# GabeTsai/YOLO-For-Turbines

Hardware: AMD Instinct MI355X
Metric: images/sec at 416x416 (fwd) (higher is better)
Workload: dtype f32; 1 GPU; BASELINE configs[1]: batch 32/GPU 416x416 fp32 inference, 80-class head, YOLOv3 forward (75 fused conv launches); per_gpu_batch=32, global_batch=32, image_size=416, num_classes=80, parallelism=image-sharded x1 (no collective)

## Files before the change

### yolo_for_turbines_amd/csrc/conv_wino4_f32.hip

```cpp
#include "wino_dma.h"

namespace yolo {

__device__ constexpr float W4_BT[6][6] = {
    {1.f, 1.5f, -2.f, -1.5f, 1.f, 0.f},
    {0.f, -1.f, -2.5f, -0.5f, 1.f, 0.f},
    {0.f, 1.f, 0.5f, -2.5f, 1.f, 0.f},
    {0.f, -0.5f, -1.f, 0.5f, 1.f, 0.f},
    {0.f, 2.f, -1.f, -2.f, 1.f, 0.f},
    {0.f, 1.f, 1.5f, -2.f, -1.5f, 1.f},
};
__device__ constexpr float W4_AT[4][6] = {
    {1.f, 1.f, 1.f, 1.f, 1.f, 0.f},
    {0.f, 1.f, -1.f, 2.f, -0.5f, 0.f},
    {0.f, 1.f, 1.f, 4.f, 0.25f, 0.f},
    {0.f, 1.f, -1.f, 8.f, -0.125f, 1.f},
};
__device__ constexpr double W4_G[6][3] = {
    {1.0, 0.0, 0.0},
    {-1.0 / 3, -1.0 / 3, -1.0 / 3},
    {1.0 / 3, -1.0 / 3, 1.0 / 3},
    {1.0 / 15, 2.0 / 15, 4.0 / 15},
    {-16.0 / 15, 8.0 / 15, -4.0 / 15},
    {0.0, 0.0, 1.0},
};

struct Wino4XArgs {
    const float* x;
    float* V;
    int H, W, C4, C4p;
    int x_ld, x_off;
    int th, tw, T, Tpad;
    int ncg;
    int nxb;
    const float* w;
    float* U;
    int cout, cin, coutp, cinp, kpad;
    long long utotal;
};

__device__ __forceinline__ void wino4_filter_elems(const Wino4XArgs& p, long long first, long long stride) {
    for (long long i = first; i < p.utotal; i += stride) {
        const int e = (int)(i & 3);
        const long long r = i >> 2;
        const int co = (int)(r % p.coutp), c4 = (int)(r / p.coutp);
        const int ci = 4 * c4 + e;
        double g[3][3];
        const bool ok = co < p.cout && ci < p.cin;
#pragma unroll
        for (int k = 0; k < 9; ++k) g[k / 3][k % 3] = ok ? (double)p.w[(size_t)co * p.kpad + k * p.cinp + ci] : 0.0;
        double t[6][3];
#pragma unroll
        for (int j = 0; j < 6; ++j)
#pragma unroll
            for (int q = 0; q < 3; ++q) t[j][q] = W4_G[j][0] * g[0][q] + W4_G[j][1] * g[1][q] + W4_G[j][2] * g[2][q];
        float* dst = p.U + i;
        const size_t xs = (size_t)p.C4p * p.coutp * 4;
#pragma unroll
        for (int j = 0; j < 6; ++j)
#pragma unroll
            for (int l = 0; l < 6; ++l)
                dst[(6 * j + l) * xs] = (float)(t[j][0] * W4_G[l][0] + t[j][1] * W4_G[l][1] + t[j][2] * W4_G[l][2]);
    }
}

__global__ __launch_bounds__(256) void wino4_filters_f32(const Wino4XArgs p) {
    wino4_filter_elems(p, (long long)blockIdx.x * blockDim.x + threadIdx.x, (long long)gridDim.x * blockDim.x);
}

__global__ __launch_bounds__(256) void wino4_xform_f32(const Wino4XArgs p) {
    if ((int)blockIdx.x >= p.nxb) {
        wino4_filter_elems(p, (long long)(blockIdx.x - p.nxb) * blockDim.x + threadIdx.x, (long long)(gridDim.x - p.nxb) * blockDim.x);
        return;
    }
    const int lane = threadIdx.x & 63, wave = threadIdx.x >> 6;
    const int cg = blockIdx.x % p.ncg, tb = blockIdx.x / p.ncg;
    const int c4 = cg * 8 + (lane & 7);
    const int t = tb * 32 + wave * 8 + (lane >> 3);
    if (c4 >= p.C4p) return;
    const bool tv = t < p.T && c4 < p.C4;
    const int tt = t < p.T ? t : 0;
    const int per = p.th * p.tw;
    const int n = tt / per, rem = tt - n * per;
    const int ty = rem / p.tw, tx = rem - ty * p.tw;
    const int r0 = 4 * ty - 1, c0 = 4 * tx - 1;
    const float* base = p.x + p.x_off + 4 * (c4 < p.C4 ? c4 : 0);
    f32x4 v[6][6];
#pragma unroll
    for (int i = 0; i < 6; ++i)
#pragma unroll
        for (int l = 0; l < 6; ++l) v[i][l] = f32x4{0.f, 0.f, 0.f, 0.f};
#pragma unroll
    for (int k = 0; k < 6; ++k) {
        const int r = r0 + k;
        const bool rv = tv && r >= 0 && r < p.H;
        f32x4 d[6];
#pragma unroll
        for (int j = 0; j < 6; ++j) {
            const int c = c0 + j;
            const bool ok = rv && c >= 0 && c < p.W;
            const size_t pix = ok ? ((size_t)n * p.H + r) * p.W + c : 0;
            const f32x4 ld = *reinterpret_cast<const f32x4*>(base + pix * p.x_ld);
            const f32x4 z = {0.f, 0.f, 0.f, 0.f};
            d[j] = ok ? ld : z;
        }
        f32x4 e[6];
#pragma unroll
        for (int l = 0; l < 6; ++l) {
            e[l] = f32x4{0.f, 0.f, 0.f, 0.f};
#pragma unroll
            for (int j = 0; j < 6; ++j)
                if (W4_BT[l][j] != 0.f) e[l] += W4_BT[l][j] * d[j];
        }
#pragma unroll
        for (int i = 0; i < 6; ++i)
            if (W4_BT[i][k] != 0.f)
#pragma unroll
                for (int l = 0; l < 6; ++l) v[i][l] += W4_BT[i][k] * e[l];
    }
    float* dst = p.V + ((size_t)c4 * p.Tpad + t) * 4;
    const size_t xs = (size_t)p.C4p * p.Tpad * 4;
#pragma unroll
    for (int i = 0; i < 6; ++i)
#pragma unroll
        for (int l = 0; l < 6; ++l) *reinterpret_cast<f32x4*>(dst + (6 * i + l) * xs) = v[i][l];
}

struct Wino4Args {
    const float* V;
    const float* U;
    const float* scale;
    const float* shift;
    const float* res;
    float* y;
    int* nan_flag;
    int T, Tpad, C4p, Cout, CoutPad;
    int th, tw, H, W;
    int y_ld, y_off, r_ld, r_off;
    int flags;
    int n_mt, n_nt;
    int n_whole;
};

constexpr int W4_STAGE = 24576;
constexpr int W4_SLOTS = 4;
constexpr int W4_DMA = 3;
constexpr int W4_TAB = 512;

template <int OFF>
__device__ __forceinline__ void w4_read3(float& a, float& b0, float& b1, unsigned ua, unsigned va) {
    asm volatile("ds_read_b32 %0, %1 offset:%2" : "=&v"(a) : "v"(ua), "n"(OFF));
    asm volatile("ds_read_b32 %0, %1 offset:%2" : "=&v"(b0) : "v"(va), "n"(OFF));
    asm volatile("ds_read_b32 %0, %1 offset:%2" : "=&v"(b1) : "v"(va), "n"(OFF + 256));
}

template <int ACT, bool RES>
__global__ __launch_bounds__(512, 1) void conv_wino4_f32(const Wino4Args p) {
    extern __shared__ __attribute__((aligned(16))) char smem[];
    const int tid = threadIdx.x, lane = tid & 63;
    const int wave = __builtin_amdgcn_readfirstlane(tid >> 6);
    const int l16 = lane & 15, kq = lane >> 4;
    const int xcd = blockIdx.x & 7, q = blockIdx.x >> 3;
    const int nt = q % p.n_nt, row = q / p.n_nt;
    const int wrows = (p.n_whole + 7) >> 3;
    const bool cut = row >= wrows;
    const int half = (row - wrows) & 1;
    const int mt = cut ? p.n_whole + ((row - wrows) >> 1) * 8 + xcd : row * 8 + xcd;
    if (mt >= (cut ? p.n_mt : p.n_whole)) return;
    const int wm = cut ? half : wave & 1, wn = cut ? wave & 3 : wave >> 1;
    const bool busy = !cut || wave < 4;

    int* tab = reinterpret_cast<int*>(smem + W4_SLOTS * W4_STAGE);
    if (tid < 64) {
        const int t = mt * 64 + tid;
        const bool tv = t < p.T && (!cut || (tid >> 5) == half);
        const int tt = tv ? t : 0;
        const int per = p.th * p.tw;
        const int n = tt / per, rem = tt - n * per;
        const int ty = rem / p.tw, tx = rem - ty * p.tw;
        const int nr = p.H - 4 * ty < 4 ? p.H - 4 * ty : 4, nc = p.W - 4 * tx < 4 ? p.W - 4 * tx : 4;
        tab[tid] = (n * p.H + 4 * ty) * p.W + 4 * tx;
        tab[64 + tid] = tv ? (nr << 4 | nc) : 0;
    }

    const size_t v_xi = (size_t)p.C4p * p.Tpad * 4, v_c4 = (size_t)p.Tpad * 4;
    const size_t u_xi = (size_t)p.C4p * p.CoutPad * 4, u_c4 = (size_t)p.CoutPad * 4;
    const int grp = wave >> 1, x0 = 3 * (wave & 1);
    const int plane = grp & 1;
    const char* src = grp < 2 ? reinterpret_cast<const char*>(p.V + plane * v_c4 + (size_t)mt * 256)
                              : reinterpret_cast<const char*>(p.U + plane * u_c4 + (size_t)nt * 256);
    const size_t s_xi = (grp < 2 ? v_xi : u_xi) * 4, s_c4 = (grp < 2 ? v_c4 : u_c4) * 4;
    const unsigned lane16 = lane * 16;
    const unsigned lds0 = (unsigned)(size_t)(wn_lptr)smem;
    auto issue_piece = [&](int k, int pass, int st, int slot) {
        const int x = x0 + k;
        wn_glds16_s(src + (size_t)(6 * pass + x) * s_xi + (size_t)(2 * st) * s_c4, lane16, lds0 + slot * W4_STAGE + (6 * grp + x) * 1024);
    };
    auto issue = [&](int pass, int st, int slot) { wn_for<0, W4_DMA>([&](auto K) { issue_piece(decltype(K)::value, pass, st, slot); }); };

    const unsigned vb = lds0 + (32 * wm + l16) * 16 + kq * 4;
    const unsigned ub = lds0 + 12288 + (16 * wn + l16) * 16 + kq * 4;

    const int nst = p.C4p / 2;
    f32x4 py[2][4][4];
#pragma unroll
    for (int bb = 0; bb < 2; ++bb)
#pragma unroll
        for (int i = 0; i < 4; ++i)
#pragma unroll
            for (int j = 0; j < 4; ++j) py[bb][i][j] = f32x4{0.f, 0.f, 0.f, 0.f};

    auto run_pass = [&](auto PASS) {
        constexpr int a = decltype(PASS)::value;
        float fa[12], fb0[12], fb1[12];
        if constexpr (a == 0) {
            issue(0, 0, 0);
            if (nst > 1) issue(0, 1, 1);
            if (nst > 2) issue(0, 2, 2);
        }
        __builtin_amdgcn_sched_barrier(0);
        f32x4 acc[6][2];
#pragma unroll
        for (int x = 0; x < 6; ++x)
#pragma unroll
            for (int bb = 0; bb < 2; ++bb) acc[x][bb] = f32x4{0.f, 0.f, 0.f, 0.f};
#pragma unroll
        for (int x = 0; x < 6; ++x) asm volatile("" : "+v"(acc[x][0]), "+v"(acc[x][1]));
        __builtin_amdgcn_sched_barrier(0);
        if (nst > 2) wn_wait_vmcnt<2 * W4_DMA>();
        else if (nst > 1) wn_wait_vmcnt<W4_DMA>();
        else wn_wait_vmcnt<0>();
        __builtin_amdgcn_s_barrier();
        __builtin_amdgcn_sched_barrier(0);
        w4_read3<0>(fa[0], fb0[0], fb1[0], ub, vb);
        w4_read3<1024>(fa[1], fb0[1], fb1[1], ub, vb);

        int slot = 0;
        for (int st = 0; st < nst; ++st) {
            const unsigned sb = (unsigned)slot * W4_STAGE;
            const int ns = (slot + 1) & (W4_SLOTS - 1);
            const unsigned nb = (unsigned)ns * W4_STAGE;
            wn_for<0, 12>([&](auto S) {
                constexpr int s = decltype(S)::value, x = s % 6;
                if constexpr (s == 10) {
                    __builtin_amdgcn_sched_barrier(0);
                    if (st + 2 < nst) wn_wait_vmcnt<W4_DMA>();
                    else wn_wait_vmcnt<0>();
                    __builtin_amdgcn_s_barrier();
                    __builtin_amdgcn_sched_barrier(0);
                }
                if constexpr (s + 2 < 12) w4_read3<(s + 2) * 1024>(fa[s + 2], fb0[s + 2], fb1[s + 2], ub + sb, vb + sb);
                constexpr int after = s < 10 ? 6 : 3;
                asm volatile("s_waitcnt lgkmcnt(%3)" : "+v"(fa[s]), "+v"(fb0[s]), "+v"(fb1[s]) : "n"(after));
                acc[x][0] = __builtin_amdgcn_mfma_f32_16x16x4f32(fa[s], fb0[s], acc[x][0], 0, 0, 0);
                acc[x][1] = __builtin_amdgcn_mfma_f32_16x16x4f32(fa[s], fb1[s], acc[x][1], 0, 0, 0);
                if constexpr (s < W4_DMA) {
                    __builtin_amdgcn_sched_barrier(0);
                    if (st >= 1 && st + 2 < nst) issue_piece(s, a, st + 2, (slot + 2) & (W4_SLOTS - 1));
                    __builtin_amdgcn_sched_barrier(0);
                }
                if constexpr (s >= 10) {
                    __builtin_amdgcn_sched_barrier(0);
                    w4_read3<(s - 10) * 1024>(fa[s - 10], fb0[s - 10], fb1[s - 10], ub + nb, vb + nb);
                    __builtin_amdgcn_sched_barrier(0);
                }
            });
            slot = ns;
        }
        asm volatile("s_waitcnt lgkmcnt(0)" ::: "memory");
        __syncthreads();
        if constexpr (a < 5) {
            issue(a + 1, 0, 0);
            if (nst > 1) issue(a + 1, 1, 1);
            if (nst > 2) issue(a + 1, 2, 2);
            __builtin_amdgcn_sched_barrier(0);
        }
#pragma unroll
        for (int bb = 0; bb < 2; ++bb) {
            f32x4 mb[6];
#pragma unroll
            for (int b = 0; b < 6; ++b) mb[b] = acc[b][bb];
            f32x4 t[4];
#pragma unroll
            for (int j = 0; j < 4; ++j) {
                t[j] = f32x4{0.f, 0.f, 0.f, 0.f};
#pragma unroll
                for (int b = 0; b < 6; ++b)
                    if (W4_AT[j][b] != 0.f) t[j] += W4_AT[j][b] * mb[b];
            }
#pragma unroll
            for (int i = 0; i < 4; ++i)
                if (W4_AT[i][a] != 0.f)
#pragma unroll
                    for (int j = 0; j < 4; ++j) py[bb][i][j] += W4_AT[i][a] * t[j];
        }
#pragma unroll
        for (int bb = 0; bb < 2; ++bb)
#pragma unroll
            for (int i = 0; i < 4; ++i)
#pragma unroll
                for (int j = 0; j < 4; ++j) asm volatile("" : "+a"(py[bb][i][j]));
    };
    if (busy) {
        run_pass(std::integral_constant<int, 0>{});
        run_pass(std::integral_constant<int, 1>{});
        run_pass(std::integral_constant<int, 2>{});
        run_pass(std::integral_constant<int, 3>{});
        run_pass(std::integral_constant<int, 4>{});
        run_pass(std::integral_constant<int, 5>{});
    } else {
        for (int a = 0; a < 6; ++a) {
            if (a == 0) {
                issue(0, 0, 0);
                if (nst > 1) issue(0, 1, 1);
                if (nst > 2) issue(0, 2, 2);
            }
            if (nst > 2) wn_wait_vmcnt<2 * W4_DMA>();
            else if (nst > 1) wn_wait_vmcnt<W4_DMA>();
            else wn_wait_vmcnt<0>();
            __builtin_amdgcn_s_barrier();
            int slot = 0;
            for (int st = 0; st < nst; ++st) {
                if (st >= 1 && st + 2 < nst) issue(a, st + 2, (slot + 2) & (W4_SLOTS - 1));
                if (st + 2 < nst) wn_wait_vmcnt<W4_DMA>();
                else wn_wait_vmcnt<0>();
                __builtin_amdgcn_s_barrier();
                slot = (slot + 1) & (W4_SLOTS - 1);
            }
            __syncthreads();
            if (a < 5) {
                issue(a + 1, 0, 0);
                if (nst > 1) issue(a + 1, 1, 1);
                if (nst > 2) issue(a + 1, 2, 2);
            }
        }
    }

    constexpr int OLD = 68;
    float* ost = reinterpret_cast<float*>(smem);
    const int c16 = tid & 15;
    const int co_t = nt * 64 + 4 * c16;
    const bool cv = co_t < p.Cout;
    const f32x4 sc_t = *reinterpret_cast<const f32x4*>(p.scale + (cv ? co_t : 0));
    const f32x4 sh_t = *reinterpret_cast<const f32x4*>(p.shift + (cv ? co_t : 0));
    auto row_pixels = [&](int i, int (&pix)[8], bool (&pv)[8]) {
#pragma unroll
        for (int it = 0; it < 8; ++it) {
            const int tl = (tid >> 4) + 32 * (it & 1), j = it >> 1;
            const int fl = tab[64 + tl];
            pv[it] = cv && j < (fl & 15) && i < (fl >> 4);
            pix[it] = pv[it] ? tab[tl] + i * p.W + j : 0;
        }
    };
    auto request_res = [&](const int (&pix)[8], f32x4 (&rr)[8]) {
#pragma unroll
        for (int it = 0; it < 8; ++it)
            rr[it] = *reinterpret_cast<const f32x4*>(p.res + (size_t)pix[it] * p.r_ld + p.r_off + (cv ? co_t : 0));
    };
    f32x4 rr[8];
    if (RES) {
        int pix[8];
        bool pv[8];
        row_pixels(0, pix, pv);
        request_res(pix, rr);
    }
    __builtin_amdgcn_sched_barrier(0);
    bool saw_nan = false;
#pragma unroll
    for (int i = 0; i < 4; ++i) {
        if (i > 0) __syncthreads();
        if (busy) {
            float* dst = ost + (32 * wm + l16) * OLD + 16 * wn + 4 * kq;
#pragma unroll
            for (int bb = 0; bb < 2; ++bb)
#pragma unroll
                for (int j = 0; j < 4; ++j) *reinterpret_cast<f32x4*>(dst + (j * 64 + 16 * bb) * OLD) = py[bb][i][j];
        }
        __syncthreads();
        int pix[8];
        bool pv[8];
        row_pixels(i, pix, pv);
        f32x4 va[8];
#pragma unroll
        for (int it = 0; it < 8; ++it)
            va[it] = *reinterpret_cast<const f32x4*>(ost + ((it >> 1) * 64 + (tid >> 4) + 32 * (it & 1)) * OLD + 4 * c16);
#pragma unroll
        for (int it = 0; it < 8; ++it) {
#pragma unroll
            for (int e = 0; e < 4; ++e) va[it][e] = act_c<ACT>(va[it][e] * sc_t[e] + sh_t[e]);
            if (RES) va[it] += rr[it];
            saw_nan |= pv[it] & ((va[it][0] != va[it][0]) | (va[it][1] != va[it][1]) | (va[it][2] != va[it][2]) | (va[it][3] != va[it][3]));
        }
#pragma unroll
        for (int it = 0; it < 8; ++it) asm volatile("" : "+v"(va[it]));
        if (RES && i < 3) {
            int npix[8];
            bool npv[8];
            row_pixels(i + 1, npix, npv);
            request_res(npix, rr);
            __builtin_amdgcn_sched_barrier(0);
        }
#pragma unroll
        for (int it = 0; it < 8; ++it)
            if (pv[it]) *reinterpret_cast<f32x4*>(p.y + (size_t)pix[it] * p.y_ld + p.y_off + co_t) = va[it];
    }
    if ((p.flags & YOLO_FLAG_NANCHECK) && saw_nan) atomicOr(p.nan_flag, 2);
}

static long long wino4_tiles(const yolo_conv_desc* d) { return (long long)d->n * ((d->h + 3) / 4) * ((d->w + 3) / 4); }

bool wino4_supported(const yolo_conv_desc* d) {
    if (!wino_supported(d)) return false;
    const long long T = wino4_tiles(d);
    if (T + 64 > 0x7fffffffLL / 4) return false;
    const long long C4p = (d->cin / 4 + 1) / 2 * 2, ncg = (C4p + 7) / 8;
    return (T + 63) / 32 * ncg + 1024 <= 0x7fffffffLL;
}

bool wino4_eligible(const yolo_conv_desc* d) {
    if (switches().no_winograd || !wino_eligible(d) || !wino4_supported(d)) return false;
    const long long area = (long long)d->h * d->w, padded = 16LL * ((d->h + 3) / 4) * ((d->w + 3) / 4);
    return area >= 26 * 26 && 5 * padded <= 6 * area;
}

size_t wino4_workspace_bytes(const yolo_conv_desc* d) {
    if (!wino4_supported(d)) return 0;
    const size_t C4p = (size_t)(d->cin / 4 + 1) / 2 * 2;
    const size_t Tpad = (size_t)(wino4_tiles(d) + 63) / 64 * 64;
    const size_t CoutPad = (size_t)round_up(d->cout, 64);
    return 36 * C4p * (Tpad + CoutPad) * 4 * sizeof(float);
}

static int wino4_num_cus() {
    static std::atomic<int> cus[64];
    int dev = 0;
    if (hipGetDevice(&dev) != hipSuccess) { (void)hipGetLastError(); return 0; }
    int n = cus[dev & 63].load(std::memory_order_relaxed);
    if (n > 0) return n;
    if (hipDeviceGetAttribute(&n, hipDeviceAttributeMultiprocessorCount, dev) != hipSuccess || n <= 0) { (void)hipGetLastError(); return 0; }
    cus[dev & 63].store(n, std::memory_order_relaxed);
    return n;
}

static int wino4_whole_blocks(int n_mt, int n_nt, int cus) {
    if (cus <= 0) return n_mt;
    const long long wgs = (long long)n_mt * n_nt;
    const int whole = (int)(wgs / cus * cus / n_nt);
    const long long tail = (long long)(n_mt - whole) * n_nt;
    return tail == 0 || 2 * tail > cus ? n_mt : whole;
}

static void wino4_filter_args(Wino4XArgs& xa, const yolo_conv_desc* d, const float* w_rm, float* U) {
    const int C4p = round_up(d->cin / 4, 2), CoutPad = round_up(d->cout, 64);
    xa.C4p = C4p;
    xa.w = w_rm; xa.U = U; xa.cout = d->cout; xa.cin = d->cin; xa.coutp = CoutPad; xa.cinp = cin_pad_of(d->cin); xa.kpad = kpad_of(d->cin, 3);
    xa.utotal = (long long)C4p * CoutPad * 4;
}
static int wino4_filter_blocks(const Wino4XArgs& xa) {
    const long long ub = (xa.utotal + 255) / 256;
    return (int)(ub < 1024 ? ub : 1024);
}

size_t wino4_filter_bytes(const yolo_conv_desc* d) {
    if (!wino4_supported(d)) return 0;
    return (size_t)36 * round_up(d->cin / 4, 2) * round_up(d->cout, 64) * 4 * sizeof(float);
}

int conv_wino4_launch(const yolo_conv_desc* d, const void* x, const float* w_rm, const float* U4_ready, const float* scale, const float* shift,
                      const void* residual, void* y, void* workspace, size_t workspace_bytes, int32_t* nan_flag, hipStream_t s) {
    if (!wino4_supported(d)) return fail(YOLO_ERR_UNSUPPORTED, "conv winograd F(4x4): needs fp32 3x3 stride 1, NHWC output, channels %% 4 == 0");
    const size_t need = wino4_workspace_bytes(d);
    if (!workspace || workspace_bytes < need) return fail(YOLO_ERR_WORKSPACE, "conv winograd F(4x4): workspace %zu < %zu bytes", workspace_bytes, need);
    if ((size_t)workspace & 15) return fail(YOLO_ERR_ARG, "conv winograd F(4x4): workspace must be 16-byte aligned");
    if ((size_t)U4_ready & 15) return fail(YOLO_ERR_ARG, "conv winograd F(4x4): transformed filters must be 16-byte aligned");
    const int th = (d->h + 3) / 4, tw = (d->w + 3) / 4;
    const int T = d->n * th * tw, Tpad = round_up(T, 64), C4 = d->cin / 4, C4p = round_up(C4, 2);
    const int CoutPad = round_up(d->cout, 64);
    float* V = (float*)workspace;
    float* U = V + (size_t)36 * C4p * Tpad * 4;
    Wino4XArgs xa;
    wino4_filter_args(xa, d, w_rm, U);
    xa.x = (const float*)x; xa.V = V; xa.H = d->h; xa.W = d->w; xa.C4 = C4; xa.x_ld = d->x_ld; xa.x_off = d->x_off;
    xa.th = th; xa.tw = tw; xa.T = T; xa.Tpad = Tpad; xa.ncg = ceil_div(C4p, 8);
    xa.nxb = (Tpad / 32) * xa.ncg;
    const int nub = U4_ready ? 0 : wino4_filter_blocks(xa);
    hipLaunchKernelGGL(wino4_xform_f32, dim3((unsigned)(xa.nxb + nub)), dim3(256), 0, s, xa);
    if (int rc = check_launch("wino4_xform_f32")) return rc;

    Wino4Args a;
    a.V = V; a.U = U4_ready ? U4_ready : U; a.scale = scale; a.shift = shift; a.res = (const float*)residual; a.y = (float*)y;
    a.nan_flag = nan_flag;
    a.T = T; a.Tpad = Tpad; a.C4p = C4p; a.Cout = d->cout; a.CoutPad = CoutPad;
    a.th = th; a.tw = tw; a.H = d->h; a.W = d->w;
    a.y_ld = d->y_ld; a.y_off = d->y_off; a.r_ld = d->r_ld; a.r_off = d->r_off; a.flags = d->flags;
    a.n_mt = Tpad / 64; a.n_nt = CoutPad / 64;
    a.n_whole = wino4_whole_blocks(a.n_mt, a.n_nt, wino4_num_cus());
    const int grid = 8 * a.n_nt * (ceil_div(a.n_whole, 8) + 2 * ceil_div(a.n_mt - a.n_whole, 8));
    const bool res = d->flags & YOLO_FLAG_RESIDUAL;
    const size_t lds = (size_t)W4_SLOTS * W4_STAGE + W4_TAB;
    auto go = [&](auto kern) -> int {
        static LdsOnce once;
        if (int rc = reserve_lds(once, reinterpret_cast<const void*>(kern), lds, "conv_wino4_f32")) return rc;
        hipLaunchKernelGGL(kern, dim3(grid), dim3(512), lds, s, a);
        return check_launch("conv_wino4_f32");
    };
    YOLO_SWITCH_ACT(d->act, return res ? go(&conv_wino4_f32<ACT, true>) : go(&conv_wino4_f32<ACT, false>));
    return fail(YOLO_ERR_ARG, "conv winograd F(4x4): activation");
}

}

extern "C" {

size_t yolo_wino4_filter_bytes(const yolo_conv_desc* d) { return d ? yolo::wino4_filter_bytes(d) : 0; }

int yolo_wino4_filters(const yolo_conv_desc* d, const void* w_packed, void* U4, void* stream) {
    using namespace yolo;
    if (!d || !w_packed || !U4) return fail(YOLO_ERR_ARG, "wino4 filters: null pointer");
    if (!wino4_supported(d)) return fail(YOLO_ERR_UNSUPPORTED, "wino4 filters: needs fp32 3x3 stride 1, NHWC output, channels %% 4 == 0");
    if ((size_t)U4 & 15) return fail(YOLO_ERR_ARG, "wino4 filters: U4 must be 16-byte aligned");
    Wino4XArgs xa{};
    wino4_filter_args(xa, d, (const float*)w_packed, (float*)U4);
    hipLaunchKernelGGL(wino4_filters_f32, dim3((unsigned)wino4_filter_blocks(xa)), dim3(256), 0, (hipStream_t)stream, xa);
    return check_launch("wino4_filters_f32");
}

int yolo_conv_wino4_blocks(const yolo_conv_desc* d, int* whole, int* half) {
    using namespace yolo;
    if (!d || !whole || !half) return fail(YOLO_ERR_ARG, "wino4 blocks: null pointer");
    if (!wino4_supported(d)) return fail(YOLO_ERR_UNSUPPORTED, "wino4 blocks: needs fp32 3x3 stride 1, NHWC output, channels %% 4 == 0");
    const int cus = wino4_num_cus();
    if (cus <= 0) return fail(YOLO_ERR_LAUNCH, "wino4 blocks: no current device");
    const int n_mt = (int)((wino4_tiles(d) + 63) / 64), n_nt = round_up(d->cout, 64) / 64;
    *whole = wino4_whole_blocks(n_mt, n_nt, cus);
    *half = n_mt - *whole;
    return YOLO_OK;
}

}
```

Baseline: 2853 images/s.

## Use all eight waves on cut Winograd F(4,3) tiles with single-column MFMA work

For the partial (cut) M-tiles, the old kernel left four of eight waves idle except for DMA and barrier participation. Now every wave computes a 16-row slice with one MFMA column (NB=1), templating the pass and epilogue on NB. This spreads the 32-tile half across all waves and drops the duplicated idle-wave control path. The cost is extra code instantiation, register pressure from two variants, and lane ids recomputed via mbcnt to limit live ranges.

```diff
diff --git a/yolo_for_turbines_amd/csrc/conv_wino4_f32.hip b/yolo_for_turbines_amd/csrc/conv_wino4_f32.hip
--- a/yolo_for_turbines_amd/csrc/conv_wino4_f32.hip
+++ b/yolo_for_turbines_amd/csrc/conv_wino4_f32.hip
@@ -147,11 +147,11 @@
 constexpr int W4_DMA = 3;
 constexpr int W4_TAB = 512;
 
-template <int OFF>
-__device__ __forceinline__ void w4_read3(float& a, float& b0, float& b1, unsigned ua, unsigned va) {
+template <int OFF, int NB>
+__device__ __forceinline__ void w4_read(float& a, float& b0, float& b1, unsigned ua, unsigned va) {
     asm volatile("ds_read_b32 %0, %1 offset:%2" : "=&v"(a) : "v"(ua), "n"(OFF));
     asm volatile("ds_read_b32 %0, %1 offset:%2" : "=&v"(b0) : "v"(va), "n"(OFF));
-    asm volatile("ds_read_b32 %0, %1 offset:%2" : "=&v"(b1) : "v"(va), "n"(OFF + 256));
+    if constexpr (NB == 2) asm volatile("ds_read_b32 %0, %1 offset:%2" : "=&v"(b1) : "v"(va), "n"(OFF + 256));
 }
 
 template <int ACT, bool RES>
@@ -167,8 +167,7 @@
     const int half = (row - wrows) & 1;
     const int mt = cut ? p.n_whole + ((row - wrows) >> 1) * 8 + xcd : row * 8 + xcd;
     if (mt >= (cut ? p.n_mt : p.n_whole)) return;
-    const int wm = cut ? half : wave & 1, wn = cut ? wave & 3 : wave >> 1;
-    const bool busy = !cut || wave < 4;
+    const int trow = cut ? 32 * half + 16 * (wave >> 2) : 32 * (wave & 1), wn = cut ? wave & 3 : wave >> 1;
 
     int* tab = reinterpret_cast<int*>(smem + W4_SLOTS * W4_STAGE);
     if (tid < 64) {
@@ -190,50 +189,46 @@
     const char* src = grp < 2 ? reinterpret_cast<const char*>(p.V + plane * v_c4 + (size_t)mt * 256)
                               : reinterpret_cast<const char*>(p.U + plane * u_c4 + (size_t)nt * 256);
     const size_t s_xi = (grp < 2 ? v_xi : u_xi) * 4, s_c4 = (grp < 2 ? v_c4 : u_c4) * 4;
-    const unsigned lane16 = lane * 16;
     const unsigned lds0 = (unsigned)(size_t)(wn_lptr)smem;
+    unsigned lane16 = lane * 16;
     auto issue_piece = [&](int k, int pass, int st, int slot) {
         const int x = x0 + k;
         wn_glds16_s(src + (size_t)(6 * pass + x) * s_xi + (size_t)(2 * st) * s_c4, lane16, lds0 + slot * W4_STAGE + (6 * grp + x) * 1024);
     };
     auto issue = [&](int pass, int st, int slot) { wn_for<0, W4_DMA>([&](auto K) { issue_piece(decltype(K)::value, pass, st, slot); }); };
 
-    const unsigned vb = lds0 + (32 * wm + l16) * 16 + kq * 4;
+    const unsigned vb = lds0 + (trow + l16) * 16 + kq * 4;
     const unsigned ub = lds0 + 12288 + (16 * wn + l16) * 16 + kq * 4;
 
     const int nst = p.C4p / 2;
-    f32x4 py[2][4][4];
-#pragma unroll
-    for (int bb = 0; bb < 2; ++bb)
-#pragma unroll
-        for (int i = 0; i < 4; ++i)
-#pragma unroll
-            for (int j = 0; j < 4; ++j) py[bb][i][j] = f32x4{0.f, 0.f, 0.f, 0.f};
-
-    auto run_pass = [&](auto PASS) {
+    auto run_pass = [&](auto PASS, auto& py) {
         constexpr int a = decltype(PASS)::value;
+        constexpr int NB = (int)std::extent<std::remove_reference_t<decltype(py)>>::value;
         float fa[12], fb0[12], fb1[12];
+        lane16 = 16u * __builtin_amdgcn_mbcnt_hi(~0u, __builtin_amdgcn_mbcnt_lo(~0u, 0u));
         if constexpr (a == 0) {
             issue(0, 0, 0);
             if (nst > 1) issue(0, 1, 1);
             if (nst > 2) issue(0, 2, 2);
         }
         __builtin_amdgcn_sched_barrier(0);
-        f32x4 acc[6][2];
+        f32x4 acc[6][NB];
 #pragma unroll
         for (int x = 0; x < 6; ++x)
 #pragma unroll
-            for (int bb = 0; bb < 2; ++bb) acc[x][bb] = f32x4{0.f, 0.f, 0.f, 0.f};
-#pragma unroll
-        for (int x = 0; x < 6; ++x) asm volatile("" : "+v"(acc[x][0]), "+v"(acc[x][1]));
+            for (int bb = 0; bb < NB; ++bb) acc[x][bb] = f32x4{0.f, 0.f, 0.f, 0.f};
+#pragma unroll
+        for (int x = 0; x < 6; ++x)
+#pragma unroll
+            for (int bb = 0; bb < NB; ++bb) asm volatile("" : "+v"(acc[x][bb]));
         __builtin_amdgcn_sched_barrier(0);
         if (nst > 2) wn_wait_vmcnt<2 * W4_DMA>();
         else if (nst > 1) wn_wait_vmcnt<W4_DMA>();
         else wn_wait_vmcnt<0>();
         __builtin_amdgcn_s_barrier();
         __builtin_amdgcn_sched_barrier(0);
-        w4_read3<0>(fa[0], fb0[0], fb1[0], ub, vb);
-        w4_read3<1024>(fa[1], fb0[1], fb1[1], ub, vb);
+        w4_read<0, NB>(fa[0], fb0[0], fb1[0], ub, vb);
+        w4_read<1024, NB>(fa[1], fb0[1], fb1[1], ub, vb);
 
         int slot = 0;
         for (int st = 0; st < nst; ++st) {
@@ -249,11 +244,12 @@
                     __builtin_amdgcn_s_barrier();
                     __builtin_amdgcn_sched_barrier(0);
                 }
-                if constexpr (s + 2 < 12) w4_read3<(s + 2) * 1024>(fa[s + 2], fb0[s + 2], fb1[s + 2], ub + sb, vb + sb);
-                constexpr int after = s < 10 ? 6 : 3;
-                asm volatile("s_waitcnt lgkmcnt(%3)" : "+v"(fa[s]), "+v"(fb0[s]), "+v"(fb1[s]) : "n"(after));
+                if constexpr (s + 2 < 12) w4_read<(s + 2) * 1024, NB>(fa[s + 2], fb0[s + 2], fb1[s + 2], ub + sb, vb + sb);
+                constexpr int after = (s < 10 ? 2 : 1) * (1 + NB);
+                if constexpr (NB == 2) asm volatile("s_waitcnt lgkmcnt(%3)" : "+v"(fa[s]), "+v"(fb0[s]), "+v"(fb1[s]) : "n"(after));
+                else asm volatile("s_waitcnt lgkmcnt(%2)" : "+v"(fa[s]), "+v"(fb0[s]) : "n"(after));
                 acc[x][0] = __builtin_amdgcn_mfma_f32_16x16x4f32(fa[s], fb0[s], acc[x][0], 0, 0, 0);
-                acc[x][1] = __builtin_amdgcn_mfma_f32_16x16x4f32(fa[s], fb1[s], acc[x][1], 0, 0, 0);
+                if constexpr (NB == 2) acc[x][1] = __builtin_amdgcn_mfma_f32_16x16x4f32(fa[s], fb1[s], acc[x][1], 0, 0, 0);
                 if constexpr (s < W4_DMA) {
                     __builtin_amdgcn_sched_barrier(0);
                     if (st >= 1 && st + 2 < nst) issue_piece(s, a, st + 2, (slot + 2) & (W4_SLOTS - 1));
@@ -261,7 +257,7 @@
                 }
                 if constexpr (s >= 10) {
                     __builtin_amdgcn_sched_barrier(0);
-                    w4_read3<(s - 10) * 1024>(fa[s - 10], fb0[s - 10], fb1[s - 10], ub + nb, vb + nb);
+                    w4_read<(s - 10) * 1024, NB>(fa[s - 10], fb0[s - 10], fb1[s - 10], ub + nb, vb + nb);
                     __builtin_amdgcn_sched_barrier(0);
                 }
             });
@@ -276,7 +272,7 @@
             __builtin_amdgcn_sched_barrier(0);
         }
 #pragma unroll
-        for (int bb = 0; bb < 2; ++bb) {
+        for (int bb = 0; bb < NB; ++bb) {
             f32x4 mb[6];
 #pragma unroll
             for (int b = 0; b < 6; ++b) mb[b] = acc[b][bb];
@@ -294,115 +290,107 @@
 #pragma unroll
                     for (int j = 0; j < 4; ++j) py[bb][i][j] += W4_AT[i][a] * t[j];
         }
-#pragma unroll
-        for (int bb = 0; bb < 2; ++bb)
+        if constexpr (a < 5 || NB == 2)
+#pragma unroll
+        for (int bb = 0; bb < NB; ++bb)
 #pragma unroll
             for (int i = 0; i < 4; ++i)
 #pragma unroll
                 for (int j = 0; j < 4; ++j) asm volatile("" : "+a"(py[bb][i][j]));
     };
-    if (busy) {
-        run_pass(std::integral_constant<int, 0>{});
-        run_pass(std::integral_constant<int, 1>{});
-        run_pass(std::integral_constant<int, 2>{});
-        run_pass(std::integral_constant<int, 3>{});
-        run_pass(std::integral_constant<int, 4>{});
-        run_pass(std::integral_constant<int, 5>{});
-    } else {
-        for (int a = 0; a < 6; ++a) {
-            if (a == 0) {
-                issue(0, 0, 0);
-                if (nst > 1) issue(0, 1, 1);
-                if (nst > 2) issue(0, 2, 2);
-            }
-            if (nst > 2) wn_wait_vmcnt<2 * W4_DMA>();
-            else if (nst > 1) wn_wait_vmcnt<W4_DMA>();
-            else wn_wait_vmcnt<0>();
-            __builtin_amdgcn_s_barrier();
-            int slot = 0;
-            for (int st = 0; st < nst; ++st) {
-                if (st >= 1 && st + 2 < nst) issue(a, st + 2, (slot + 2) & (W4_SLOTS - 1));
-                if (st + 2 < nst) wn_wait_vmcnt<W4_DMA>();
-                else wn_wait_vmcnt<0>();
-                __builtin_amdgcn_s_barrier();
-                slot = (slot + 1) & (W4_SLOTS - 1);
-            }
-            __syncthreads();
-            if (a < 5) {
-                issue(a + 1, 0, 0);
-                if (nst > 1) issue(a + 1, 1, 1);
-                if (nst > 2) issue(a + 1, 2, 2);
-            }
-        }
-    }
+    auto run_passes = [&](auto& py) {
+        constexpr int NB = (int)std::extent<std::remove_reference_t<decltype(py)>>::value;
+#pragma unroll
+        for (int bb = 0; bb < NB; ++bb)
+#pragma unroll
+            for (int i = 0; i < 4; ++i)
+#pragma unroll
+                for (int j = 0; j < 4; ++j) py[bb][i][j] = f32x4{0.f, 0.f, 0.f, 0.f};
+        wn_for<0, 6>([&](auto PASS) { run_pass(PASS, py); });
+    };
 
     constexpr int OLD = 68;
     float* ost = reinterpret_cast<float*>(smem);
-    const int c16 = tid & 15;
-    const int co_t = nt * 64 + 4 * c16;
-    const bool cv = co_t < p.Cout;
-    const f32x4 sc_t = *reinterpret_cast<const f32x4*>(p.scale + (cv ? co_t : 0));
-    const f32x4 sh_t = *reinterpret_cast<const f32x4*>(p.shift + (cv ? co_t : 0));
-    auto row_pixels = [&](int i, int (&pix)[8], bool (&pv)[8]) {
-#pragma unroll
-        for (int it = 0; it < 8; ++it) {
-            const int tl = (tid >> 4) + 32 * (it & 1), j = it >> 1;
-            const int fl = tab[64 + tl];
-            pv[it] = cv && j < (fl & 15) && i < (fl >> 4);
-            pix[it] = pv[it] ? tab[tl] + i * p.W + j : 0;
+    bool saw_nan = false;
+    auto epilogue = [&](auto& py) {
+        constexpr int NB = (int)std::extent<std::remove_reference_t<decltype(py)>>::value;
+        constexpr int NIT = 4 * NB;
+        const int lane = __builtin_amdgcn_mbcnt_hi(~0u, __builtin_amdgcn_mbcnt_lo(~0u, 0u));
+        const int tid = wave * 64 + lane, l16 = lane & 15, kq = lane >> 4;
+        const int c16 = tid & 15;
+        const int co_t = nt * 64 + 4 * c16;
+        const bool cv = co_t < p.Cout;
+        const f32x4 sc_t = *reinterpret_cast<const f32x4*>(p.scale + (cv ? co_t : 0));
+        const f32x4 sh_t = *reinterpret_cast<const f32x4*>(p.shift + (cv ? co_t : 0));
+        auto tile_of = [&](int it) { return NB == 2 ? (tid >> 4) + 32 * (it & 1) : (tid >> 4) + 32 * half; };
+        auto pixel_of = [&](int it) { return NB == 2 ? it >> 1 : it; };
+        auto row_pixels = [&](int i, int (&pix)[NIT], bool (&pv)[NIT]) {
+#pragma unroll
+            for (int it = 0; it < NIT; ++it) {
+                const int tl = tile_of(it), j = pixel_of(it);
+                const int fl = tab[64 + tl];
+                pv[it] = cv && j < (fl & 15) && i < (fl >> 4);
+                pix[it] = pv[it] ? tab[tl] + i * p.W + j : 0;
+            }
+        };
+        auto request_res = [&](const int (&pix)[NIT], f32x4 (&rr)[NIT]) {
+#pragma unroll
+            for (int it = 0; it < NIT; ++it)
+                rr[it] = *reinterpret_cast<const f32x4*>(p.res + (size_t)pix[it] * p.r_ld + p.r_off + (cv ? co_t : 0));
+        };
+        f32x4 rr[NIT];
+        if (RES) {
+            int pix[NIT];
+            bool pv[NIT];
+            row_pixels(0, pix, pv);
+            request_res(pix, rr);
+        }
+        __builtin_amdgcn_sched_barrier(0);
+#pragma unroll
+        for (int i = 0; i < 4; ++i) {
+            if (i > 0) __syncthreads();
+            float* dst = ost + (trow + l16) * OLD + 16 * wn + 4 * kq;
+#pragma unroll
+            for (int bb = 0; bb < NB; ++bb)
+#pragma unroll
+                for (int j = 0; j < 4; ++j) *reinterpret_cast<f32x4*>(dst + (j * 64 + 16 * bb) * OLD) = py[bb][i][j];
+            __syncthreads();
+            int pix[NIT];
+            bool pv[NIT];
+            row_pixels(i, pix, pv);
+            f32x4 va[NIT];
+#pragma unroll
+            for (int it = 0; it < NIT; ++it)
+                va[it] = *reinterpret_cast<const f32x4*>(ost + (pixel_of(it) * 64 + tile_of(it)) * OLD + 4 * c16);
+#pragma unroll
+            for (int it = 0; it < NIT; ++it) {
+#pragma unroll
+                for (int e = 0; e < 4; ++e) va[it][e] = act_c<ACT>(va[it][e] * sc_t[e] + sh_t[e]);
+                if (RES) va[it] += rr[it];
+                saw_nan |= pv[it] & ((va[it][0] != va[it][0]) | (va[it][1] != va[it][1]) | (va[it][2] != va[it][2]) | (va[it][3] != va[it][3]));
+            }
+#pragma unroll
+            for (int it = 0; it < NIT; ++it) asm volatile("" : "+v"(va[it]));
+            if (RES && i < 3) {
+                int npix[NIT];
+                bool npv[NIT];
+                row_pixels(i + 1, npix, npv);
+                request_res(npix, rr);
+                __builtin_amdgcn_sched_barrier(0);
+            }
+#pragma unroll
+            for (int it = 0; it < NIT; ++it)
+                if (pv[it]) *reinterpret_cast<f32x4*>(p.y + (size_t)pix[it] * p.y_ld + p.y_off + co_t) = va[it];
         }
     };
-    auto request_res = [&](const int (&pix)[8], f32x4 (&rr)[8]) {
-#pragma unroll
-        for (int it = 0; it < 8; ++it)
-            rr[it] = *reinterpret_cast<const f32x4*>(p.res + (size_t)pix[it] * p.r_ld + p.r_off + (cv ? co_t : 0));
-    };
-    f32x4 rr[8];
-    if (RES) {
-        int pix[8];
-        bool pv[8];
-        row_pixels(0, pix, pv);
-        request_res(pix, rr);
-    }
-    __builtin_amdgcn_sched_barrier(0);
-    bool saw_nan = false;
-#pragma unroll
-    for (int i = 0; i < 4; ++i) {
-        if (i > 0) __syncthreads();
-        if (busy) {
-            float* dst = ost + (32 * wm + l16) * OLD + 16 * wn + 4 * kq;
-#pragma unroll
-            for (int bb = 0; bb < 2; ++bb)
-#pragma unroll
-                for (int j = 0; j < 4; ++j) *reinterpret_cast<f32x4*>(dst + (j * 64 + 16 * bb) * OLD) = py[bb][i][j];
-        }
-        __syncthreads();
-        int pix[8];
-        bool pv[8];
-        row_pixels(i, pix, pv);
-        f32x4 va[8];
-#pragma unroll
-        for (int it = 0; it < 8; ++it)
-            va[it] = *reinterpret_cast<const f32x4*>(ost + ((it >> 1) * 64 + (tid >> 4) + 32 * (it & 1)) * OLD + 4 * c16);
-#pragma unroll
-        for (int it = 0; it < 8; ++it) {
-#pragma unroll
-            for (int e = 0; e < 4; ++e) va[it][e] = act_c<ACT>(va[it][e] * sc_t[e] + sh_t[e]);
-            if (RES) va[it] += rr[it];
-            saw_nan |= pv[it] & ((va[it][0] != va[it][0]) | (va[it][1] != va[it][1]) | (va[it][2] != va[it][2]) | (va[it][3] != va[it][3]));
-        }
-#pragma unroll
-        for (int it = 0; it < 8; ++it) asm volatile("" : "+v"(va[it]));
-        if (RES && i < 3) {
-            int npix[8];
-            bool npv[8];
-            row_pixels(i + 1, npix, npv);
-            request_res(npix, rr);
-            __builtin_amdgcn_sched_barrier(0);
-        }
-#pragma unroll
-        for (int it = 0; it < 8; ++it)
-            if (pv[it]) *reinterpret_cast<f32x4*>(p.y + (size_t)pix[it] * p.y_ld + p.y_off + co_t) = va[it];
+    if (cut) {
+        f32x4 py[1][4][4];
+        run_passes(py);
+        epilogue(py);
+    } else {
+        f32x4 py[2][4][4];
+        run_passes(py);
+        epilogue(py);
     }
     if ((p.flags & YOLO_FLAG_NANCHECK) && saw_nan) atomicOr(p.nan_flag, 2);
 }
```

Result: no change. 2831 images/s (-0.8%).
